# askerlee/AdaFace-dev

Measured on AMD Instinct MI355X. Metric: denoise-steps/sec SD-1.5 U-Net 512px bs=4/GPU, higher is better.
Workload: dtype f16; 1 GPU; adaface_txt2img_ddim: SD-1.5 U-Net eps-prediction + CFG + DDIM update, 512x512 (latent 64x64), bs=4/GPU, U-Net batch 8 (cond+uncond), 77 tokens, DDIM-50 timesteps, random-init weights; parallelism=replicas x1, hipgraph=True, finite=True

## Files before the change

adaface-dev_amd/csrc/af_attn.hip:

```cpp
#include <float.h>
#include <stdlib.h>

#include "af_common.h"

namespace {

struct AttnArgs {
  const half_t* q;
  const half_t* k;
  const half_t* vt;
  half_t* o;
  const float* kbias;
  float* lse2;
  int ld_lse;
  int causal_m;
  int B, Nq, L, heads, d;
  int ldq, ldk, ldo, ldv, ldb;
  long vbs;
  float c;
};

constexpr int KB = 64;
constexpr int VST = 36;
constexpr float kLazy = 8.0f;

template <int DS, bool ONES, bool GENERAL>
__global__ __launch_bounds__(256) void af_attn_kernel(AttnArgs a) {
  constexpr int DP = 16 * DS;
  constexpr int DT = (DS + 1) / 2;
  constexpr int DV = 32 * DT;
  constexpr int KST = DP + 8;
  constexpr int KBUF = KB * KST;
  constexpr int VBUF = 2 * DV * VST;
  constexpr int STAGE = KBUF + VBUF;
  constexpr int KCH = KB * (DP / 8);
  constexpr int NKC = (KCH + 255) / 256;
  constexpr int VCH = DV * 8;
  constexpr int NVC = (VCH + 255) / 256;
  extern __shared__ __attribute__((aligned(16))) char af_smem[];
  half_t* lds = reinterpret_cast<half_t*>(af_smem);

  const int tid = threadIdx.x, lane = tid & 63, wave = tid >> 6;
  const int r = lane & 31, hh = lane >> 5;
  const int qblocks = (a.Nq + 127) / 128;
  const int xcd = blockIdx.x & 7, idx = blockIdx.x >> 3;
  const int bh = (idx / qblocks) * 8 + xcd;
  if (bh >= a.B * a.heads) return;
  const int b = bh / a.heads, h = bh - b * a.heads;
  const int query = (idx % qblocks) * 128 + wave * 32 + r;


  half8_t qf[DS];
  const half8_t zero8 = {0, 0, 0, 0, 0, 0, 0, 0};
  {
    const half_t* qp = a.q + ((size_t)b * a.Nq + (query < a.Nq ? query : 0)) * a.ldq + h * a.d;
#pragma unroll
    for (int s = 0; s < DS; ++s) {
      const int dc = 16 * s + 8 * hh;
      half8_t v = (query < a.Nq && dc < a.d) ? *reinterpret_cast<const half8_t*>(qp + dc) : zero8;
#pragma unroll
      for (int e = 0; e < 8; ++e) v[e] = (half_t)((float)v[e] * a.c);
      qf[s] = v;
    }
  }

  half8_t rk[NKC], rv[NVC];
  const half_t* kptr[NKC];
  bool kok[NKC];
#pragma unroll
  for (int j = 0; j < NKC; ++j) {
    const int i = tid + 256 * j;
    const int row = i / (DP / 8), ch = i - row * (DP / 8);
    kok[j] = i < KCH && ch * 8 < a.d;
    kptr[j] = a.k + ((size_t)b * a.L + row) * a.ldk + h * a.d + ch * 8;
  }
  const half_t* vptr[NVC];
  bool vok[NVC], vones[NVC];
#pragma unroll
  for (int j = 0; j < NVC; ++j) {
    const int i = tid + 256 * j;
    const int row = i >> 3, ch = i & 7;
    vok[j] = i < VCH && row < a.d;
    vones[j] = ONES && i < VCH && row == DV - 1;
    vptr[j] = a.vt + (size_t)b * a.vbs + (size_t)(h * a.d + (row < a.d ? row : 0)) * a.ldv + ch * 8;
  }
  const half8_t ones8 = {1, 1, 1, 1, 1, 1, 1, 1};
  auto load_stage = [&](int key0) {
#pragma unroll
    for (int j = 0; j < NKC; ++j) {
      const int row = (tid + 256 * j) / (DP / 8);
      const bool ok = kok[j] && (!GENERAL || key0 + row < a.L);
      rk[j] = ok ? *reinterpret_cast<const half8_t*>(kptr[j] + (size_t)key0 * a.ldk) : zero8;
    }
#pragma unroll
    for (int j = 0; j < NVC; ++j) {
      const int kk = key0 + ((tid + 256 * j) & 7) * 8;
      const bool ok = vok[j] && (!GENERAL || kk < a.L);
      half8_t fill = zero8;
      if (ONES) {
        if (GENERAL) {
          if (vones[j]) {
#pragma unroll
            for (int e = 0; e < 8; ++e) fill[e] = (kk + e < a.L) ? (half_t)1 : (half_t)0;
          }
        } else {
          fill = vones[j] ? ones8 : zero8;
        }
      }
      rv[j] = ok ? *reinterpret_cast<const half8_t*>(vptr[j] + key0) : fill;
    }
  };
  auto store_stage = [&](int buf, int key0_store) {
    half_t* Ks = lds + buf * STAGE;
    half_t* Vs = Ks + KBUF;
#pragma unroll
    for (int j = 0; j < NKC; ++j) {
      const int i = tid + 256 * j;
      if (i < KCH) {
        const int row = i / (DP / 8), ch = i - row * (DP / 8);
        *reinterpret_cast<half8_t*>(Ks + row * KST + ch * 8) = rk[j];
      }
    }
#pragma unroll
    for (int j = 0; j < NVC; ++j) {
      const int i = tid + 256 * j;
      if (i < VCH) {
        const int row = i >> 3, ch = i & 7;
        half_t* dst = Vs + ((ch >> 2) * DV + row) * VST + (ch & 3) * 8;
        if (GENERAL) {
          const int kk = key0_store + ch * 8;
          if (kk + 8 > a.L) {
#pragma unroll
            for (int e = 0; e < 8; ++e)
              if (kk + e >= a.L) rv[j][e] = (half_t)0;
          }
        }
        const half4_t lo = {rv[j][0], rv[j][1], rv[j][2], rv[j][3]};
        const half4_t hi = {rv[j][4], rv[j][5], rv[j][6], rv[j][7]};
        *reinterpret_cast<half4_t*>(dst) = lo;
        *reinterpret_cast<half4_t*>(dst + 4) = hi;
      }
    }
  };

  floatx16 o[DT];
#pragma unroll
  for (int t = 0; t < DT; ++t)
#pragma unroll
    for (int i = 0; i < 16; ++i) o[t][i] = 0.f;
  float m = -FLT_MAX, l = 0.f;

  const int nstage = (a.L + KB - 1) / KB;
  load_stage(0);
  store_stage(0, 0);
  __syncthreads();
  for (int st = 0; st < nstage; ++st) {
    const int key0 = st * KB;
    const bool more = st + 1 < nstage;
    if (more) load_stage(key0 + KB);

    const half_t* Ks = lds + (st & 1) * STAGE;
    const half_t* Vs = Ks + KBUF;
    const int nsub = GENERAL ? ((key0 + 32 < a.L) ? 2 : 1) : 2;

    floatx16 sT[2];
    const float cinit = (GENERAL || st == 0) ? 0.f : -m;
#pragma unroll
    for (int sub = 0; sub < 2; ++sub) {
#pragma unroll
      for (int i = 0; i < 16; ++i) sT[sub][i] = cinit;
      if (sub < nsub) {
#pragma unroll
        for (int s = 0; s < DS; ++s) {
          const half8_t kf = *reinterpret_cast<const half8_t*>(Ks + (sub * 32 + r) * KST + 16 * s + 8 * hh);
          sT[sub] = __builtin_amdgcn_mfma_f32_32x32x16_f16(kf, qf[s], sT[sub], 0, 0, 0);
        }
      }
    }
    float mx = -FLT_MAX;
    if (GENERAL) {
#pragma unroll
      for (int sub = 0; sub < 2; ++sub) {
        if (sub < nsub) {
#pragma unroll
          for (int g = 0; g < 4; ++g) {
            const int kb = key0 + sub * 32 + 8 * g + 4 * hh;
            floatx4 bias = {0.f, 0.f, 0.f, 0.f};
            if (a.kbias) bias = *reinterpret_cast<const floatx4*>(a.kbias + (size_t)b * a.ldb + kb);
#pragma unroll
            for (int e = 0; e < 4; ++e) {
              float t = sT[sub][4 * g + e] + bias[e];
              bool vis = kb + e < a.L;
              if (a.causal_m > 0) vis = vis && ((kb + e) / a.causal_m <= query);
              t = vis ? t : -INFINITY;
              sT[sub][4 * g + e] = t;
              mx = fmaxf(mx, t);
            }
          }
        }
      }
    } else {
#pragma unroll
      for (int i = 0; i < 16; i += 2) {
        mx = fmaxf(fmaxf(mx, sT[0][i]), sT[0][i + 1]);
        mx = fmaxf(fmaxf(mx, sT[1][i]), sT[1][i + 1]);
      }
    }
    mx = fmaxf(mx, __shfl_xor(mx, 32, 64));
    if (GENERAL) {
      if (__builtin_amdgcn_ballot_w64(mx > m) != 0) {
        const float m_new = fmaxf(m, mx);
        const float alpha = __builtin_amdgcn_exp2f(m - m_new);
        m = m_new;
        if (!ONES) l *= alpha;
#pragma unroll
        for (int t = 0; t < DT; ++t)
#pragma unroll
          for (int i = 0; i < 16; ++i) o[t][i] *= alpha;
      }
      sT[0] = sT[0] - m;
      sT[1] = sT[1] - m;
    } else if (st == 0) {
      m = mx;
      sT[0] = sT[0] - m;
      sT[1] = sT[1] - m;
    } else if (__builtin_amdgcn_ballot_w64(mx > kLazy) != 0) {
      const float delta = fmaxf(mx, 0.f);
      const float alpha = __builtin_amdgcn_exp2f(-delta);
      m += delta;
      if (!ONES) l *= alpha;
#pragma unroll
      for (int t = 0; t < DT; ++t)
#pragma unroll
        for (int i = 0; i < 16; ++i) o[t][i] *= alpha;
      sT[0] = sT[0] - delta;
      sT[1] = sT[1] - delta;
    }

    half8_t pf[2][2];
#pragma unroll
    for (int sub = 0; sub < 2; ++sub) {
      if (sub < nsub) {
#pragma unroll
        for (int s2 = 0; s2 < 2; ++s2) {
#pragma unroll
          for (int j = 0; j < 8; ++j) {
            const float p = __builtin_amdgcn_exp2f(sT[sub][8 * s2 + j]);
            if (!ONES) l += p;
            pf[sub][s2][j] = (half_t)p;
          }
        }
      } else {
        pf[sub][0] = zero8;
        pf[sub][1] = zero8;
      }
    }
#pragma unroll
    for (int t = 0; t < DT; ++t) {
#pragma unroll
      for (int sub = 0; sub < 2; ++sub) {
        if (sub < nsub) {
#pragma unroll
          for (int s2 = 0; s2 < 2; ++s2) {
            const half_t* vp = Vs + (sub * DV + 32 * t + r) * VST + 16 * s2 + 4 * hh;
            const half4_t lo = *reinterpret_cast<const half4_t*>(vp);
            const half4_t hi = *reinterpret_cast<const half4_t*>(vp + 8);
            const half8_t vf = {lo[0], lo[1], lo[2], lo[3], hi[0], hi[1], hi[2], hi[3]};
            o[t] = __builtin_amdgcn_mfma_f32_32x32x16_f16(vf, pf[sub][s2], o[t], 0, 0, 0);
          }
        }
      }
    }

    if (more) store_stage((st + 1) & 1, key0 + KB);
    __syncthreads();
  }

  if (ONES) {
    const float mine = o[DT - 1][15];
    const float other = __shfl_xor(mine, 32, 64);
    l = hh ? mine : other;
  } else {
    l += __shfl_xor(l, 32, 64);
  }
  const float inv = 1.0f / l;
  if (a.lse2 && query < a.Nq && hh == 0) a.lse2[((size_t)b * a.heads + h) * a.ld_lse + query] = m + __builtin_amdgcn_logf(l);
  if (query < a.Nq) {
    half_t* op = a.o + ((size_t)b * a.Nq + query) * a.ldo + h * a.d;
#pragma unroll
    for (int t = 0; t < DT; ++t) {
#pragma unroll
      for (int g = 0; g < 4; ++g) {
        const int dd = 32 * t + 8 * g + 4 * hh;
        if (dd < a.d) {
          const half4_t v = {(half_t)(o[t][4 * g + 0] * inv), (half_t)(o[t][4 * g + 1] * inv),
                             (half_t)(o[t][4 * g + 2] * inv), (half_t)(o[t][4 * g + 3] * inv)};
          *reinterpret_cast<half4_t*>(op + dd) = v;
        }
      }
    }
  }
}

template <int DS, bool ONES, bool SLOT = false, int NW = 4>
__global__ __launch_bounds__(64 * NW) void af_attn2_kernel(AttnArgs a) {
  constexpr int NT = 64 * NW;
  constexpr int DP = 16 * DS, DT = (DS + 1) / 2, DV = 32 * DT;
  constexpr int KST = DP + 8, KBUF = KB * KST, VBUF = 2 * DV * VST, STAGE = KBUF + VBUF;
  constexpr int KCH = KB * (DP / 8), NKC = (KCH + NT - 1) / NT, VCH = DV * 8, NVC = (VCH + NT - 1) / NT;
  extern __shared__ __attribute__((aligned(16))) char af_smem[];
  half_t* lds = reinterpret_cast<half_t*>(af_smem);
  const int tid = threadIdx.x, lane = tid & 63, wave = tid >> 6;
  const int r = lane & 31, hh = lane >> 5;
  const int qblocks = (a.Nq + NT - 1) / NT;
  const int xcd = blockIdx.x & 7, idx = blockIdx.x >> 3;
  const int bh = (idx / qblocks) * 8 + xcd;
  if (bh >= a.B * a.heads) return;
  const int b = bh / a.heads, h = bh - b * a.heads;
  const int q0 = (idx % qblocks) * NT + wave * 64 + r;
  const half8_t zero8 = {0, 0, 0, 0, 0, 0, 0, 0};

  half8_t qf[2][DS];
#pragma unroll
  for (int c = 0; c < 2; ++c) {
    const int query = q0 + 32 * c;
    const half_t* qp = a.q + ((size_t)b * a.Nq + (query < a.Nq ? query : 0)) * a.ldq + h * a.d;
#pragma unroll
    for (int s = 0; s < DS; ++s) {
      const int dc = 16 * s + 8 * hh;
      half8_t v = (query < a.Nq && dc < a.d) ? *reinterpret_cast<const half8_t*>(qp + dc) : zero8;
#pragma unroll
      for (int e = 0; e < 8; ++e) v[e] = (half_t)((float)v[e] * a.c);
      qf[c][s] = v;
    }
  }

  half8_t rk[NKC], rv[NVC];
  const half_t* kptr[NKC];
  bool kok[NKC], kone[NKC];
#pragma unroll
  for (int j = 0; j < NKC; ++j) {
    const int i = tid + NT * j;
    const int row = i / (DP / 8), ch = i - row * (DP / 8);
    kok[j] = i < KCH && ch * 8 < a.d;
    kone[j] = SLOT && i < KCH && ch * 8 == a.d;
    kptr[j] = a.k + ((size_t)b * a.L + row) * a.ldk + h * a.d + ch * 8;
  }
  const half8_t one1 = {1, 0, 0, 0, 0, 0, 0, 0};
  const half_t* vptr[NVC];
  bool vok[NVC], vones[NVC];
#pragma unroll
  for (int j = 0; j < NVC; ++j) {
    const int i = tid + NT * j;
    const int row = i >> 3, ch = i & 7;
    vok[j] = i < VCH && row < a.d;
    vones[j] = ONES && i < VCH && row == DV - 1;
    vptr[j] = a.vt + (size_t)b * a.vbs + (size_t)(h * a.d + (row < a.d ? row : 0)) * a.ldv + ch * 8;
  }
  const half8_t ones8 = {1, 1, 1, 1, 1, 1, 1, 1};
  auto load_stage = [&](int key0) {
#pragma unroll
    for (int j = 0; j < NKC; ++j) rk[j] = kok[j] ? *reinterpret_cast<const half8_t*>(kptr[j] + (size_t)key0 * a.ldk) : (kone[j] ? one1 : zero8);
#pragma unroll
    for (int j = 0; j < NVC; ++j) rv[j] = vok[j] ? *reinterpret_cast<const half8_t*>(vptr[j] + key0) : (vones[j] ? ones8 : zero8);
  };
  auto store_stage = [&](int buf) {
    half_t* Ks = lds + buf * STAGE;
    half_t* Vs = Ks + KBUF;
#pragma unroll
    for (int j = 0; j < NKC; ++j) {
      const int i = tid + NT * j;
      if (i < KCH) {
        const int row = i / (DP / 8), ch = i - row * (DP / 8);
        *reinterpret_cast<half8_t*>(Ks + row * KST + ch * 8) = rk[j];
      }
    }
#pragma unroll
    for (int j = 0; j < NVC; ++j) {
      const int i = tid + NT * j;
      if (i < VCH) {
        const int row = i >> 3, ch = i & 7;
        half_t* dst = Vs + ((ch >> 2) * DV + row) * VST + (ch & 3) * 8;
        const half4_t lo = {rv[j][0], rv[j][1], rv[j][2], rv[j][3]};
        const half4_t hi = {rv[j][4], rv[j][5], rv[j][6], rv[j][7]};
        *reinterpret_cast<half4_t*>(dst) = lo;
        *reinterpret_cast<half4_t*>(dst + 4) = hi;
      }
    }
  };

  floatx16 o[2][DT];
#pragma unroll
  for (int c = 0; c < 2; ++c)
#pragma unroll
    for (int t = 0; t < DT; ++t)
#pragma unroll
      for (int i = 0; i < 16; ++i) o[c][t][i] = 0.f;
  float m[2] = {-FLT_MAX, -FLT_MAX}, l[2] = {0.f, 0.f};

  auto softmax = [&](int c, int st, floatx16 (&sT)[2], half8_t (&pf)[2][2]) {
    float mx = -FLT_MAX;
#pragma unroll
    for (int i = 0; i < 16; i += 2) {
      mx = fmaxf(fmaxf(mx, sT[0][i]), sT[0][i + 1]);
      mx = fmaxf(fmaxf(mx, sT[1][i]), sT[1][i + 1]);
    }
    if constexpr (SLOT) {
      const unsigned mb = __builtin_bit_cast(unsigned, mx);
      const auto sw = __builtin_amdgcn_permlane32_swap(mb, mb, false, false);
      mx = fmaxf(__builtin_bit_cast(float, (unsigned)sw[0]), __builtin_bit_cast(float, (unsigned)sw[1]));
    } else {
      mx = fmaxf(mx, __shfl_xor(mx, 32, 64));
    }
    if (st == 0) {
      const float m0 = SLOT ? (float)(half_t)mx : mx;
      m[c] = m0;
      sT[0] = sT[0] - m0;
      sT[1] = sT[1] - m0;
      if (SLOT && hh) qf[c][DS - 1][0] = (half_t)(-m0);
    } else if (__builtin_amdgcn_ballot_w64(mx > kLazy) != 0) {
      float delta = fmaxf(mx, 0.f);
      if constexpr (SLOT) {
        const float mn = (float)(half_t)(m[c] + delta);
        delta = mn - m[c];
        if (hh) qf[c][DS - 1][0] = (half_t)(-mn);
      }
      const float alpha = __builtin_amdgcn_exp2f(-delta);
      m[c] += delta;
      if (!ONES) l[c] *= alpha;
#pragma unroll
      for (int t = 0; t < DT; ++t)
#pragma unroll
        for (int i = 0; i < 16; ++i) o[c][t][i] *= alpha;
      sT[0] = sT[0] - delta;
      sT[1] = sT[1] - delta;
    }
#pragma unroll
    for (int sub = 0; sub < 2; ++sub)
#pragma unroll
      for (int s2 = 0; s2 < 2; ++s2)
#pragma unroll
        for (int j = 0; j < 8; ++j) {
          const float p = __builtin_amdgcn_exp2f(sT[sub][8 * s2 + j]);
          if (!ONES) l[c] += p;
          pf[sub][s2][j] = (half_t)p;
        }
  };

  const int nstage = a.L / KB;
  load_stage(0);
  store_stage(0);
  __syncthreads();
  if (NW == 8 && __builtin_amdgcn_readfirstlane(wave) >= 4) __builtin_amdgcn_s_setprio(1);
  for (int st = 0; st < nstage; ++st) {
    const bool more = st + 1 < nstage;
    if (more) load_stage((st + 1) * KB);
    const half_t* Ks = lds + (st & 1) * STAGE;
    const half_t* Vs = Ks + KBUF;

    floatx16 sA[2], sB[2];
    const floatx16 zero16 = {0.f, 0.f, 0.f, 0.f, 0.f, 0.f, 0.f, 0.f, 0.f, 0.f, 0.f, 0.f, 0.f, 0.f, 0.f, 0.f};
    if constexpr (!SLOT) {
      const float ca = st == 0 ? 0.f : -m[0], cb = st == 0 ? 0.f : -m[1];
#pragma unroll
      for (int sub = 0; sub < 2; ++sub) {
#pragma unroll
        for (int i = 0; i < 16; ++i) {
          sA[sub][i] = ca;
          sB[sub][i] = cb;
        }
      }
    }
#pragma unroll
    for (int sub = 0; sub < 2; ++sub)
#pragma unroll
      for (int s = 0; s < DS; ++s) {
        const half8_t kf = *reinterpret_cast<const half8_t*>(Ks + (sub * 32 + r) * KST + 16 * s + 8 * hh);
        sA[sub] = __builtin_amdgcn_mfma_f32_32x32x16_f16(kf, qf[0][s], (SLOT && s == 0) ? zero16 : sA[sub], 0, 0, 0);
      }
#pragma unroll
    for (int sub = 0; sub < 2; ++sub)
#pragma unroll
      for (int s = 0; s < DS; ++s) {
        const half8_t kf = *reinterpret_cast<const half8_t*>(Ks + (sub * 32 + r) * KST + 16 * s + 8 * hh);
        sB[sub] = __builtin_amdgcn_mfma_f32_32x32x16_f16(kf, qf[1][s], (SLOT && s == 0) ? zero16 : sB[sub], 0, 0, 0);
      }
    half8_t pA[2][2], pB[2][2];
    softmax(0, st, sA, pA);
#pragma unroll
    for (int t = 0; t < DT; ++t)
#pragma unroll
      for (int sub = 0; sub < 2; ++sub)
#pragma unroll
        for (int s2 = 0; s2 < 2; ++s2) {
          const half_t* vp = Vs + (sub * DV + 32 * t + r) * VST + 16 * s2 + 4 * hh;
          const half4_t lo = *reinterpret_cast<const half4_t*>(vp);
          const half4_t hi = *reinterpret_cast<const half4_t*>(vp + 8);
          const half8_t vf = {lo[0], lo[1], lo[2], lo[3], hi[0], hi[1], hi[2], hi[3]};
          o[0][t] = __builtin_amdgcn_mfma_f32_32x32x16_f16(vf, pA[sub][s2], o[0][t], 0, 0, 0);
        }
    softmax(1, st, sB, pB);
#pragma unroll
    for (int t = 0; t < DT; ++t)
#pragma unroll
      for (int sub = 0; sub < 2; ++sub)
#pragma unroll
        for (int s2 = 0; s2 < 2; ++s2) {
          const half_t* vp = Vs + (sub * DV + 32 * t + r) * VST + 16 * s2 + 4 * hh;
          const half4_t lo = *reinterpret_cast<const half4_t*>(vp);
          const half4_t hi = *reinterpret_cast<const half4_t*>(vp + 8);
          const half8_t vf = {lo[0], lo[1], lo[2], lo[3], hi[0], hi[1], hi[2], hi[3]};
          o[1][t] = __builtin_amdgcn_mfma_f32_32x32x16_f16(vf, pB[sub][s2], o[1][t], 0, 0, 0);
        }
    if (more) store_stage((st + 1) & 1);
    __syncthreads();
  }

#pragma unroll
  for (int c = 0; c < 2; ++c) {
    const int query = q0 + 32 * c;
    float lc = l[c];
    if (ONES) {
      const float mine = o[c][DT - 1][15];
      const float other = __shfl_xor(mine, 32, 64);
      lc = hh ? mine : other;
    } else {
      lc += __shfl_xor(lc, 32, 64);
    }
    const float inv = 1.0f / lc;
    if (a.lse2 && query < a.Nq && hh == 0) a.lse2[((size_t)b * a.heads + h) * a.ld_lse + query] = m[c] + __builtin_amdgcn_logf(lc);
    if (query < a.Nq) {
      half_t* op = a.o + ((size_t)b * a.Nq + query) * a.ldo + h * a.d;
#pragma unroll
      for (int t = 0; t < DT; ++t)
#pragma unroll
        for (int g = 0; g < 4; ++g) {
          const int dd = 32 * t + 8 * g + 4 * hh;
          if (dd < a.d) {
            const half4_t v = {(half_t)(o[c][t][4 * g + 0] * inv), (half_t)(o[c][t][4 * g + 1] * inv),
                               (half_t)(o[c][t][4 * g + 2] * inv), (half_t)(o[c][t][4 * g + 3] * inv)};
            *reinterpret_cast<half4_t*>(op + dd) = v;
          }
        }
    }
  }
}

template <int DS, bool ONES, bool SLOT = false>
int launch_attn2chain(const AttnArgs& a, hipStream_t stream) {
  constexpr int DP = 16 * DS, DT = (DS + 1) / 2, DV = 32 * DT;
  constexpr size_t lds = (size_t)2 * (KB * (DP + 8) + 2 * DV * VST) * sizeof(half_t);
  const int bh8 = (a.B * a.heads + 7) / 8 * 8;
  constexpr int kDefaultNw = 8;
  const char* nw_s = getenv("AF_ATTN_NW");
  const int nw = nw_s ? atoi(nw_s) : kDefaultNw;
  if (nw == 8 && SLOT && a.Nq % 512 == 0) {
    static bool attr8 = false;
    if (!af_allow_dyn_lds(reinterpret_cast<const void*>(&af_attn2_kernel<DS, ONES, SLOT, 8>), lds, attr8, "af_attention")) return af_check_launch("af_attention");
    hipLaunchKernelGGL((af_attn2_kernel<DS, ONES, SLOT, 8>), dim3((a.Nq / 512) * bh8), dim3(512), lds, stream, a);
    return af_check_launch("af_attention(two-chain, 8 waves)");
  }
  static bool attr_set = false;
  if (!af_allow_dyn_lds(reinterpret_cast<const void*>(&af_attn2_kernel<DS, ONES, SLOT>), lds, attr_set, "af_attention")) return af_check_launch("af_attention");
  const int qblocks = (a.Nq + 255) / 256;
  hipLaunchKernelGGL((af_attn2_kernel<DS, ONES, SLOT>), dim3(qblocks * bh8), dim3(256), lds, stream, a);
  return af_check_launch("af_attention(two-chain)");
}

template <int DS, bool ONES>
__global__ __launch_bounds__(256) void af_xattn_kernel(AttnArgs a, int groups_per_wave, int nchunk) {
  constexpr int DP = 16 * DS, DT = (DS + 1) / 2, DV = 32 * DT;
  constexpr int KST = DP + 8;
  constexpr int LP = 128;
  constexpr int KCH = LP * (DP / 8);
  constexpr int VCH = DV * (LP / 8);
  extern __shared__ __attribute__((aligned(16))) char af_smem[];
  half_t* Ks = reinterpret_cast<half_t*>(af_smem);
  half_t* Vs = Ks + LP * KST;

  const int tid = threadIdx.x, lane = tid & 63, wave = tid >> 6;
  const int r = lane & 31, hh = lane >> 5;
  const int xcd = blockIdx.x & 7, idx = blockIdx.x >> 3;
  const int bh = (idx / nchunk) * 8 + xcd;
  if (bh >= a.B * a.heads) return;
  const int chunk = idx % nchunk;
  const int b = bh / a.heads, h = bh - b * a.heads;

  const int nsub = (a.L + 31) >> 5;
  const half8_t zero8 = {0, 0, 0, 0, 0, 0, 0, 0};

  const int group0 = (chunk * 4 + wave) * groups_per_wave;
  auto load_q = [&](int grp, half8_t (&qf)[DS]) {
    const int query = grp * 32 + r;
    const half_t* qp = a.q + ((size_t)b * a.Nq + (query < a.Nq ? query : 0)) * a.ldq + h * a.d;
#pragma unroll
    for (int s2 = 0; s2 < DS; ++s2) {
      const int dc = 16 * s2 + 8 * hh;
      qf[s2] = (query < a.Nq && dc < a.d) ? *reinterpret_cast<const half8_t*>(qp + dc) : zero8;
    }
  };
  half8_t qraw[DS], qnext[DS];
  load_q(group0, qraw);

  {
    constexpr int NKC = (KCH + 255) / 256, NVC = (VCH + 255) / 256;
    half8_t rk[NKC], rv[NVC];
#pragma unroll
    for (int j = 0; j < NKC; ++j) {
      const int i = tid + 256 * j;
      const int row = i / (DP / 8), ch = i - row * (DP / 8);
      rk[j] = (i < KCH && row < a.L && ch * 8 < a.d)
                  ? *reinterpret_cast<const half8_t*>(a.k + ((size_t)b * a.L + row) * a.ldk + h * a.d + ch * 8) : zero8;
    }
#pragma unroll
    for (int j = 0; j < NVC; ++j) {
      const int i = tid + 256 * j;
      const int row = i >> 4, kk = (i & 15) * 8;
      rv[j] = (i < VCH && row < a.d && kk < a.L)
                  ? *reinterpret_cast<const half8_t*>(a.vt + (size_t)b * a.vbs + (size_t)(h * a.d + row) * a.ldv + kk) : zero8;
    }
#pragma unroll
    for (int j = 0; j < NKC; ++j) {
      const int i = tid + 256 * j;
      const int row = i / (DP / 8), ch = i - row * (DP / 8);
      if (i < KCH) *reinterpret_cast<half8_t*>(Ks + row * KST + ch * 8) = rk[j];
    }
#pragma unroll
    for (int j = 0; j < NVC; ++j) {
      const int i = tid + 256 * j;
      if (i < VCH) {
        const int row = i >> 4, ch = i & 15, kk = ch * 8;
        half8_t v = rv[j];
        if (row < a.d) {
          if (kk < a.L && kk + 8 > a.L) {
#pragma unroll
            for (int e = 0; e < 8; ++e)
              if (kk + e >= a.L) v[e] = (half_t)0;
          }
        } else if (ONES && row == DV - 1) {
#pragma unroll
          for (int e = 0; e < 8; ++e) v[e] = (kk + e < a.L) ? (half_t)1 : (half_t)0;
        }
        half_t* dst = Vs + ((ch >> 2) * DV + row) * VST + (ch & 3) * 8;
        const half4_t lo = {v[0], v[1], v[2], v[3]}, hi = {v[4], v[5], v[6], v[7]};
        *reinterpret_cast<half4_t*>(dst) = lo;
        *reinterpret_cast<half4_t*>(dst + 4) = hi;
      }
    }
  }
  __syncthreads();

  for (int gi = 0; gi < groups_per_wave; ++gi) {
    const int grp = group0 + gi;
    if (grp * 32 >= a.Nq) break;
    const int query = grp * 32 + r;
    if (gi + 1 < groups_per_wave) load_q(grp + 1, qnext);
    half8_t qf[DS];
#pragma unroll
    for (int s2 = 0; s2 < DS; ++s2)
#pragma unroll
      for (int e = 0; e < 8; ++e) qf[s2][e] = (half_t)((float)qraw[s2][e] * a.c);

    auto score_tile = [&](int sub) {
      floatx16 sc;
#pragma unroll
      for (int i = 0; i < 16; ++i) sc[i] = 0.f;
#pragma unroll
      for (int s2 = 0; s2 < DS; ++s2) {
        const half8_t kf = *reinterpret_cast<const half8_t*>(Ks + (sub * 32 + r) * KST + 16 * s2 + 8 * hh);
        sc = __builtin_amdgcn_mfma_f32_32x32x16_f16(kf, qf[s2], sc, 0, 0, 0);
      }
      if (sub == nsub - 1) {
#pragma unroll
        for (int i = 0; i < 16; ++i) {
          const int key = sub * 32 + 8 * (i >> 2) + 4 * hh + (i & 3);
          if (key >= a.L) sc[i] = -INFINITY;
        }
      }
      return sc;
    };
    float mx = -FLT_MAX;
#pragma unroll 1
    for (int sub = 0; sub < nsub; ++sub) {
      const floatx16 sc = score_tile(sub);
#pragma unroll
      for (int i = 0; i < 16; i += 2) mx = fmaxf(fmaxf(mx, sc[i]), sc[i + 1]);
    }
    mx = fmaxf(mx, __shfl_xor(mx, 32, 64));
    floatx16 o[DT];
#pragma unroll
    for (int t = 0; t < DT; ++t)
#pragma unroll
      for (int i = 0; i < 16; ++i) o[t][i] = 0.f;
    float l = 0.f;
#pragma unroll 1
    for (int sub = 0; sub < nsub; ++sub) {
      const floatx16 sc = score_tile(sub);
      half8_t pf[2];
#pragma unroll
      for (int s2 = 0; s2 < 2; ++s2)
#pragma unroll
        for (int j = 0; j < 8; ++j) {
          const float pv = __builtin_amdgcn_exp2f(sc[8 * s2 + j] - mx);
          if (!ONES) l += pv;
          pf[s2][j] = (half_t)pv;
        }
#pragma unroll
      for (int t = 0; t < DT; ++t)
#pragma unroll
        for (int s2 = 0; s2 < 2; ++s2) {
          const half_t* vp = Vs + (sub * DV + 32 * t + r) * VST + 16 * s2 + 4 * hh;
          const half4_t lo = *reinterpret_cast<const half4_t*>(vp);
          const half4_t hi = *reinterpret_cast<const half4_t*>(vp + 8);
          const half8_t vf = {lo[0], lo[1], lo[2], lo[3], hi[0], hi[1], hi[2], hi[3]};
          o[t] = __builtin_amdgcn_mfma_f32_32x32x16_f16(vf, pf[s2], o[t], 0, 0, 0);
        }
    }
    if (ONES) {
      const float mine = o[DT - 1][15];
      const float other = __shfl_xor(mine, 32, 64);
      l = hh ? mine : other;
    } else {
      l += __shfl_xor(l, 32, 64);
    }
    const float inv = 1.0f / l;
    if (a.lse2 && query < a.Nq && hh == 0) a.lse2[((size_t)b * a.heads + h) * a.ld_lse + query] = mx + __builtin_amdgcn_logf(l);
    if (query < a.Nq) {
      half_t* op = a.o + ((size_t)b * a.Nq + query) * a.ldo + h * a.d;
#pragma unroll
      for (int t = 0; t < DT; ++t)
#pragma unroll
        for (int g = 0; g < 4; ++g) {
          const int dd = 32 * t + 8 * g + 4 * hh;
          if (dd < a.d) {
            const half4_t v = {(half_t)(o[t][4 * g + 0] * inv), (half_t)(o[t][4 * g + 1] * inv),
                               (half_t)(o[t][4 * g + 2] * inv), (half_t)(o[t][4 * g + 3] * inv)};
            *reinterpret_cast<half4_t*>(op + dd) = v;
          }
        }
    }
    if (gi + 1 < groups_per_wave) {
#pragma unroll
      for (int s2 = 0; s2 < DS; ++s2) qraw[s2] = qnext[s2];
    }
  }
}

template <int DS, bool ONES>
int launch_xattn(const AttnArgs& a, hipStream_t stream) {
  constexpr int DP = 16 * DS, DT = (DS + 1) / 2, DV = 32 * DT;
  constexpr size_t lds = (size_t)(128 * (DP + 8) + 4 * DV * VST) * sizeof(half_t);
  static bool attr_set = false;
  if (!af_allow_dyn_lds(reinterpret_cast<const void*>(&af_xattn_kernel<DS, ONES>), lds, attr_set, "af_attention")) return af_check_launch("af_attention");
  const int groups = (a.Nq + 31) / 32;
  int gpw = groups / 32;
  gpw = gpw < 1 ? 1 : (gpw > 8 ? 8 : gpw);
  const int nchunk = (groups + 4 * gpw - 1) / (4 * gpw);
  const int bh8 = (a.B * a.heads + 7) / 8 * 8;
  hipLaunchKernelGGL((af_xattn_kernel<DS, ONES>), dim3(nchunk * bh8), dim3(256), lds, stream, a, gpw, nchunk);
  return af_check_launch("af_attention(short-key)");
}

template <int DS, bool ONES, bool GENERAL>
int launch_attn2(const AttnArgs& a, hipStream_t stream) {
  constexpr int DP = 16 * DS, DT = (DS + 1) / 2, DV = 32 * DT;
  constexpr size_t lds = (size_t)2 * (KB * (DP + 8) + 2 * DV * VST) * sizeof(half_t);
  static bool attr_set = false;
  if (!af_allow_dyn_lds(reinterpret_cast<const void*>(&af_attn_kernel<DS, ONES, GENERAL>), lds, attr_set, "af_attention")) return af_check_launch("af_attention");
  const int qblocks = (a.Nq + 127) / 128, bh8 = (a.B * a.heads + 7) / 8 * 8;
  dim3 grid(qblocks * bh8), block(256);
  hipLaunchKernelGGL((af_attn_kernel<DS, ONES, GENERAL>), grid, block, lds, stream, a);
  return af_check_launch("af_attention");
}

template <int DS>
int launch_attn(const AttnArgs& a, hipStream_t stream) {
  constexpr int DV = 32 * ((DS + 1) / 2);
  if (a.kbias == nullptr && a.causal_m == 0 && a.L <= 128)
    return DV > a.d ? launch_xattn<DS, true>(a, stream) : launch_xattn<DS, false>(a, stream);
  const bool general = a.kbias != nullptr || a.causal_m > 0 || a.L % KB != 0;
  if constexpr (DS <= 3) {
    if (!general && a.Nq >= 512) {
      if (a.d == 16 * DS - 8 && DV > a.d) return launch_attn2chain<DS, true, true>(a, stream);
      return DV > a.d ? launch_attn2chain<DS, true>(a, stream) : launch_attn2chain<DS, false>(a, stream);
    }
  }
  if (DV > a.d) return general ? launch_attn2<DS, true, true>(a, stream) : launch_attn2<DS, true, false>(a, stream);
  return general ? launch_attn2<DS, false, true>(a, stream) : launch_attn2<DS, false, false>(a, stream);
}

__global__ __launch_bounds__(256) void af_scores_kernel(const half_t* __restrict__ q, const half_t* __restrict__ k,
                                                        float* __restrict__ score, float* __restrict__ prob, int B, int Nq,
                                                        int L, int heads, int d, float scale) {
  const int lane = threadIdx.x & 63;
  const long row = (long)blockIdx.x * 4 + (threadIdx.x >> 6);
  const long nrows = (long)B * heads * Nq;
  if (row >= nrows) return;
  const int i = (int)(row % Nq);
  const int h = (int)((row / Nq) % heads);
  const int b = (int)(row / ((long)Nq * heads));
  const int C = heads * d;
  const half_t* qp = q + ((size_t)b * Nq + i) * C + h * d;
  float s[2];
#pragma unroll
  for (int jj = 0; jj < 2; ++jj) {
    const int j = lane + 64 * jj;
    float acc = 0.f;
    if (j < L) {
      const half_t* kp = k + ((size_t)b * L + j) * C + h * d;
      for (int c0 = 0; c0 < d; c0 += 8) {
        const half8_t qv = *reinterpret_cast<const half8_t*>(qp + c0);
        const half8_t kv = *reinterpret_cast<const half8_t*>(kp + c0);
#pragma unroll
        for (int e = 0; e < 8; ++e) acc += (float)qv[e] * (float)kv[e];
      }
    }
    s[jj] = j < L ? acc * scale : -INFINITY;
  }
  const float mx = af_wave_max(fmaxf(s[0], s[1]));
  const float e0 = __expf(s[0] - mx), e1 = __expf(s[1] - mx);
  const float inv = 1.0f / af_wave_sum(e0 + e1);
  float* sp = score + (size_t)row * L;
  float* pp = prob + (size_t)row * L;
  if (lane < L) {
    sp[lane] = s[0];
    pp[lane] = e0 * inv;
  }
  if (lane + 64 < L) {
    sp[lane + 64] = s[1];
    pp[lane + 64] = e1 * inv;
  }
}

}

extern "C" int af_attention_lse(const void* q, const void* k, const void* vt, void* o, void* lse2, int ld_lse,
                                const void* keybias, int B, int Nq, int L, int heads, int d, int ldq, int ldk, int ldo,
                                int ldv, int ldb, float scale, void* stream) {
  return af_attention_ex(q, k, vt, o, lse2, ld_lse, keybias, 0, B, Nq, L, heads, d, ldq, ldk, ldo, ldv, ldb, scale, stream);
}

extern "C" int af_attention_strided(const void* q, const void* k, const void* vt, void* o, void* lse2, int ld_lse, const void* keybias,
                                    int causal_m, int B, int Nq, int L, int heads, int d, int ldq, int ldk, int ldo, int ldv, int ldb,
                                    int64_t vt_batch_stride, float scale, void* stream);

extern "C" int af_attention_ex(const void* q, const void* k, const void* vt, void* o, void* lse2, int ld_lse,
                               const void* keybias, int causal_m, int B, int Nq, int L, int heads, int d, int ldq, int ldk,
                               int ldo, int ldv, int ldb, float scale, void* stream) {
  return af_attention_strided(q, k, vt, o, lse2, ld_lse, keybias, causal_m, B, Nq, L, heads, d, ldq, ldk, ldo, ldv, ldb,
                              (int64_t)heads * d * ldv, scale, stream);
}

extern "C" int af_attention_strided(const void* q, const void* k, const void* vt, void* o, void* lse2, int ld_lse, const void* keybias,
                                    int causal_m, int B, int Nq, int L, int heads, int d, int ldq, int ldk, int ldo, int ldv, int ldb,
                                    int64_t vt_batch_stride, float scale, void* stream) {
  AF_REQUIRE(q && k && vt && o, "af_attention: null pointer");
  AF_REQUIRE(vt_batch_stride >= (int64_t)heads * d * ldv && vt_batch_stride % 8 == 0, "af_attention: vt_batch_stride must cover heads*d rows of ldv and keep 16-byte alignment");
  AF_REQUIRE(B > 0 && Nq > 0 && L > 0 && heads > 0 && d > 0, "af_attention: bad sizes");
  AF_REQUIRE(d % 8 == 0, "af_attention: head dim must be a multiple of 8");
  AF_SUPPORTED(d <= 160, "af_attention: head dim > 160");
  const int C = heads * d;
  AF_REQUIRE(ldq >= C && ldk >= C && ldo >= C && ldq % 8 == 0 && ldk % 8 == 0 && ldo % 4 == 0,
             "af_attention: bad row strides");
  AF_REQUIRE(ldv % 8 == 0 && ldv >= ((L + 7) / 8) * 8, "af_attention: ldv must be a multiple of 8 and >= roundup(L, 8)");
  if (keybias) AF_REQUIRE(ldb >= ((L + KB - 1) / KB) * KB && ldb % 4 == 0, "af_attention: ldb must cover L rounded up to 64");
  AttnArgs a;
  a.q = (const half_t*)q;
  a.k = (const half_t*)k;
  a.vt = (const half_t*)vt;
  a.o = (half_t*)o;
  a.kbias = (const float*)keybias;
  a.lse2 = (float*)lse2;
  a.ld_lse = ld_lse;
  a.causal_m = causal_m;
  AF_REQUIRE(causal_m >= 0, "af_attention: causal_m < 0");
  if (lse2) AF_REQUIRE(ld_lse >= Nq, "af_attention: ld_lse < Nq");
  a.B = B;
  a.Nq = Nq;
  a.L = L;
  a.heads = heads;
  a.d = d;
  a.ldq = ldq;
  a.ldk = ldk;
  a.ldo = ldo;
  a.ldv = ldv;
  a.ldb = ldb;
  a.vbs = vt_batch_stride;
  a.c = scale * 1.4426950408889634f;
  AfLaunchScope scope(L < Nq ? AF_FAM_XATTN : AF_FAM_ATTN, stream);
  hipStream_t s = (hipStream_t)stream;
  const int ds = (d + 15) / 16;
  switch (ds) {
    case 1: return launch_attn<1>(a, s);
    case 2: return launch_attn<2>(a, s);
    case 3: return launch_attn<3>(a, s);
    case 4: return launch_attn<4>(a, s);
    case 5: return launch_attn<5>(a, s);
    case 6: return launch_attn<6>(a, s);
    case 8: return launch_attn<8>(a, s);
    case 10: return launch_attn<10>(a, s);
    default: return af_fail(AF_E_UNSUPPORTED, "af_attention: unsupported head dim (need ceil(d/16) in {1,2,3,4,5,6,8,10})");
  }
}

extern "C" int af_attention(const void* q, const void* k, const void* vt, void* o, const void* keybias, int B, int Nq,
                            int L, int heads, int d, int ldq, int ldk, int ldo, int ldv, int ldb, float scale,
                            void* stream) {
  return af_attention_lse(q, k, vt, o, nullptr, 0, keybias, B, Nq, L, heads, d, ldq, ldk, ldo, ldv, ldb, scale, stream);
}

extern "C" int af_attention_scores(const void* q, const void* k, void* score, void* prob, int B, int Nq, int L, int heads,
                                   int d, float scale, void* stream) {
  AF_REQUIRE(q && k && score && prob, "af_attention_scores: null pointer");
  AF_REQUIRE(B > 0 && Nq > 0 && L > 0 && heads > 0 && d > 0 && d % 8 == 0, "af_attention_scores: bad sizes");
  AF_SUPPORTED(L <= 128, "af_attention_scores: L > 128 (capture path is for cross-attention only)");
  const long rows = (long)B * heads * Nq;
  dim3 grid((unsigned)((rows + 3) / 4)), block(256);
  AfLaunchScope scope(AF_FAM_ATTN, stream);
  hipLaunchKernelGGL(af_scores_kernel, grid, block, 0, (hipStream_t)stream, (const half_t*)q, (const half_t*)k,
                     (float*)score, (float*)prob, B, Nq, L, heads, d, scale);
  return af_check_launch("af_attention_scores");
}
```

adaface-dev_amd/csrc/af_common.h:

```cpp
#pragma once
#include <hip/hip_runtime.h>
#include <stdint.h>
#include <stdlib.h>
#include <string>

#include "../../include/adaface_hip.h"

typedef _Float16 half_t;
typedef _Float16 half2_t __attribute__((ext_vector_type(2)));
typedef _Float16 half4_t __attribute__((ext_vector_type(4)));
typedef _Float16 half8_t __attribute__((ext_vector_type(8)));
typedef float floatx4 __attribute__((ext_vector_type(4)));
typedef unsigned int uintx4_t __attribute__((ext_vector_type(4)));
typedef float floatx16 __attribute__((ext_vector_type(16)));

#define AF_WAVE 64

void af_set_error(const std::string& msg);
int af_fail(int code, const std::string& msg);

struct AfLaunchScope {
  int family;
  hipStream_t stream;
  hipEvent_t ev_stop;
  unsigned epoch;
  AfLaunchScope(int family, void* stream);
  ~AfLaunchScope();
};
int af_check_launch(const char* what);
bool af_allow_dyn_lds(const void* kernel, size_t bytes, bool& done, const char* what);
void af_launch_transpose_tokens(const _Float16* x, _Float16* y, int B, int N, int C, int ldx, int ldy, hipStream_t stream);
struct AfTransposeJob {
  const _Float16* x;
  _Float16* y;
  int N, C, ldx, ldy;
};
void af_launch_transpose_tokens_multi(const AfTransposeJob* jobs, int n, int B, hipStream_t stream);

#define AF_REQUIRE(cond, msg)                                      \
  do {                                                             \
    if (!(cond)) return af_fail(AF_E_BADARG, std::string(msg));    \
  } while (0)
#define AF_SUPPORTED(cond, msg)                                      \
  do {                                                               \
    if (!(cond)) return af_fail(AF_E_UNSUPPORTED, std::string(msg)); \
  } while (0)

__device__ __forceinline__ float af_sigmoid(float x) { return __builtin_amdgcn_rcpf(1.0f + __expf(-x)); }
__device__ __forceinline__ float af_silu(float x) { return x * af_sigmoid(x); }
__device__ __forceinline__ float af_erf(float x) {
  const float ax = fabsf(x);
  const float t = __builtin_amdgcn_rcpf(fmaf(0.3275911f, ax, 1.0f));
  float p = fmaf(1.061405429f, t, -1.453152027f);
  p = fmaf(p, t, 1.421413741f);
  p = fmaf(p, t, -0.284496736f);
  p = fmaf(p, t, 0.254829592f);
  const float e = __builtin_amdgcn_exp2f(ax * ax * -1.4426950408889634f);
  return copysignf(fmaf(-p * t, e, 1.0f), x);
}
__device__ __forceinline__ float af_gelu_erf(float x) { return 0.5f * x * (1.0f + af_erf(x * 0.70710678118654752f)); }

__device__ __forceinline__ float af_wave_sum(float v) {
#pragma unroll
  for (int off = 32; off > 0; off >>= 1) v += __shfl_xor(v, off, 64);
  return v;
}
__device__ __forceinline__ float af_wave_max(float v) {
#pragma unroll
  for (int off = 32; off > 0; off >>= 1) v = fmaxf(v, __shfl_xor(v, off, 64));
  return v;
}

struct GnAcc {
  float n, s, m2;
};
__device__ __forceinline__ GnAcc gn_acc_merge(const GnAcc a, const GnAcc b) {
  if (b.n <= 0.f) return a;
  if (a.n <= 0.f) return b;
  const float n = a.n + b.n;
  const float d = b.s * __builtin_amdgcn_rcpf(b.n) - a.s * __builtin_amdgcn_rcpf(a.n);
  GnAcc r;
  r.n = n;
  r.s = a.s + b.s;
  r.m2 = a.m2 + b.m2 + d * d * (a.n * b.n * __builtin_amdgcn_rcpf(n));
  return r;
}
__device__ __forceinline__ GnAcc gn_acc_from_shifted(float n, float p, float s1, float q1) {
  GnAcc r;
  r.n = n;
  r.s = n * p + s1;
  r.m2 = n > 0.f ? fmaxf(q1 - s1 * s1 * __builtin_amdgcn_rcpf(n), 0.f) : 0.f;
  return r;
}

__device__ __forceinline__ half2_t gn_half_diff(const half2_t x, const half2_t nhp) {
  const half2_t h = {(half_t)0.5f, (half_t)0.5f};
  return x * h + nhp;
}

constexpr int AF_WPF_MAX = 8;
constexpr int AF_WPF_DUMP_BYTES = 256;
struct AfWpf {
  int budget, coop;
};
inline AfWpf af_wpf_config(int tiles_m) {
  static const int budget_env = getenv("AF_GEMM3_WPREFETCH") ? atoi(getenv("AF_GEMM3_WPREFETCH")) : 4;
  static const int coop_env = getenv("AF_GEMM3_WPF_COOP") ? atoi(getenv("AF_GEMM3_WPF_COOP")) : 32;
  return AfWpf{budget_env > AF_WPF_MAX ? AF_WPF_MAX : budget_env, tiles_m < coop_env ? tiles_m : coop_env};
}
__device__ __forceinline__ void af_prefetch_weight_tile(const half_t* wt, int kpad, int npad, int row0, int rows, int kt0, int nk, int coop, int me,
                                                        int budget, int nw, int wave, int lane, char* lds_dump) {
  const int total = rows * nk;
  const int per = (total + coop - 1) / coop;
  const int begin = me * per;
  const int end = min(total, begin + min(per, budget * nw * 64));
#pragma unroll
  for (int j = 0; j < AF_WPF_MAX; ++j) {
    const int line = begin + (j * nw + wave) * 64 + lane;
    if (j < budget && line < end) {
      const int st = line / rows, row = line - st * rows;
      const int n = row0 + row;
      if (n < npad)
        __builtin_amdgcn_global_load_lds((const __attribute__((address_space(1))) void*)(wt + (size_t)n * kpad + (size_t)(kt0 + st) * 64),
                                         (__attribute__((address_space(3))) void*)lds_dump, 4, 0, 0);
    }
  }
}
```

adaface-dev_amd/csrc/af_runtime.hip:

```cpp
#include <atomic>
#include <mutex>
#include <vector>

#include "af_common.h"

static thread_local std::string g_last_error;

void af_set_error(const std::string& msg) { g_last_error = msg; }
int af_fail(int code, const std::string& msg) {
  g_last_error = msg;
  return code;
}

extern "C" const char* af_last_error(void) { return g_last_error.c_str(); }
extern "C" int af_version(void) { return 100; }

extern "C" int af_device_count(void) {
  int n = 0;
  hipError_t e = hipGetDeviceCount(&n);
  if (e != hipSuccess) return af_fail(AF_E_HIP, std::string("hipGetDeviceCount: ") + hipGetErrorString(e));
  return n;
}

static thread_local std::string g_pending_error;

bool af_allow_dyn_lds(const void* kernel, size_t bytes, bool& done, const char* what) {
  if (done || bytes <= 65536) return true;
  hipError_t e = hipFuncSetAttribute(kernel, hipFuncAttributeMaxDynamicSharedMemorySize, (int)bytes);
  if (e != hipSuccess) {
    (void)hipGetLastError();
    g_pending_error = std::string(what) + ": hipFuncSetAttribute(MaxDynamicSharedMemorySize = " + std::to_string(bytes) + "): " + hipGetErrorString(e);
    return false;
  }
  done = true;
  return true;
}

int af_check_launch(const char* what) {
  if (!g_pending_error.empty()) {
    std::string m;
    m.swap(g_pending_error);
    (void)hipGetLastError();
    return af_fail(AF_E_HIP, m);
  }
  hipError_t e = hipGetLastError();
  if (e != hipSuccess) return af_fail(AF_E_HIP, std::string(what) + ": " + hipGetErrorString(e));
  return AF_OK;
}

namespace {
struct ProfState {
  std::mutex mu;
  std::atomic<bool> on{false};
  unsigned epoch = 0;
  struct Pair {
    hipEvent_t a, b;
  };
  std::vector<Pair> pairs[AF_FAM_COUNT];
  std::vector<Pair> pool;
};
ProfState& prof() {
  static ProfState s;
  return s;
}
}

AfLaunchScope::AfLaunchScope(int family_, void* stream_) : family(family_), stream((hipStream_t)stream_), ev_stop(nullptr), epoch(0) {
  ProfState& p = prof();
  if (!p.on.load(std::memory_order_relaxed)) return;
  hipStreamCaptureStatus cs = hipStreamCaptureStatusNone;
  if (hipStreamIsCapturing(stream, &cs) != hipSuccess || cs != hipStreamCaptureStatusNone) return;
  std::lock_guard<std::mutex> lk(p.mu);
  ProfState::Pair pr;
  if (!p.pool.empty()) {
    pr = p.pool.back();
    p.pool.pop_back();
  } else {
    if (hipEventCreate(&pr.a) != hipSuccess) return;
    if (hipEventCreate(&pr.b) != hipSuccess) {
      (void)hipEventDestroy(pr.a);
      return;
    }
  }
  (void)hipEventRecord(pr.a, stream);
  p.pairs[family].push_back(pr);
  ev_stop = pr.b;
  epoch = p.epoch;
}

AfLaunchScope::~AfLaunchScope() {
  if (!ev_stop) return;
  ProfState& p = prof();
  std::lock_guard<std::mutex> lk(p.mu);
  if (epoch != p.epoch) return;
  (void)hipEventRecord(ev_stop, stream);
}

extern "C" int af_prof_enable(int on) {
  ProfState& p = prof();
  p.on.store(on != 0);
  return AF_OK;
}

extern "C" int af_prof_reset(void) {
  ProfState& p = prof();
  std::lock_guard<std::mutex> lk(p.mu);
  ++p.epoch;
  for (int f = 0; f < AF_FAM_COUNT; ++f) {
    for (auto& pr : p.pairs[f]) p.pool.push_back(pr);
    p.pairs[f].clear();
  }
  return AF_OK;
}

extern "C" int af_prof_read(int family, int* launches, double* total_ms) {
  if (family < 0 || family >= AF_FAM_COUNT || !launches || !total_ms) return af_fail(AF_E_BADARG, "af_prof_read: bad argument");
  ProfState& p = prof();
  std::lock_guard<std::mutex> lk(p.mu);
  double tot = 0.0;
  for (auto& pr : p.pairs[family]) {
    hipError_t e = hipEventSynchronize(pr.b);
    if (e != hipSuccess) return af_fail(AF_E_HIP, std::string("hipEventSynchronize: ") + hipGetErrorString(e));
    float ms = 0.f;
    e = hipEventElapsedTime(&ms, pr.a, pr.b);
    if (e != hipSuccess) return af_fail(AF_E_HIP, std::string("hipEventElapsedTime: ") + hipGetErrorString(e));
    tot += ms;
  }
  *launches = (int)p.pairs[family].size();
  *total_ms = tot;
  return AF_OK;
}
```

Baseline: 100.1 denoise-steps/s.

## Add key-group multi-stage LDS buffering and reuse V fragments across query chains

Adds an optional attention kernel variant that stages several key blocks per barrier and prefetches K fragments into registers. It is selectable through AF_ATTN_KGROUP and defaults to off. In the default path, V fragments read from LDS for the first query chain are now kept in registers and reused for the second chain, halving V LDS reads. The trade-off is higher register pressure, which may reduce occupancy or cause spills.

```diff
diff --git a/adaface-dev_amd/csrc/af_attn.hip b/adaface-dev_amd/csrc/af_attn.hip
--- a/adaface-dev_amd/csrc/af_attn.hip
+++ b/adaface-dev_amd/csrc/af_attn.hip
@@ -1,5 +1,7 @@
 #include <float.h>
 #include <stdlib.h>
+
+#include <type_traits>
 
 #include "af_common.h"
 
@@ -302,8 +304,9 @@
   }
 }
 
-template <int DS, bool ONES, bool SLOT = false, int NW = 4>
+template <int DS, bool ONES, bool SLOT = false, int NW = 4, int KG = 1>
 __global__ __launch_bounds__(64 * NW) void af_attn2_kernel(AttnArgs a) {
+  static_assert(KG == 1 || KG == 2 || KG == 4, "key groups of 1, 2 or 4 sub-stages");
   constexpr int NT = 64 * NW;
   constexpr int DP = 16 * DS, DT = (DS + 1) / 2, DV = 32 * DT;
   constexpr int KST = DP + 8, KBUF = KB * KST, VBUF = 2 * DV * VST, STAGE = KBUF + VBUF;
@@ -398,7 +401,7 @@
       for (int i = 0; i < 16; ++i) o[c][t][i] = 0.f;
   float m[2] = {-FLT_MAX, -FLT_MAX}, l[2] = {0.f, 0.f};
 
-  auto softmax = [&](int c, int st, floatx16 (&sT)[2], half8_t (&pf)[2][2]) {
+  auto softmax = [&](int c, auto first, floatx16 (&sT)[2], half8_t (&pf)[2][2]) {
     float mx = -FLT_MAX;
 #pragma unroll
     for (int i = 0; i < 16; i += 2) {
@@ -412,7 +415,7 @@
     } else {
       mx = fmaxf(mx, __shfl_xor(mx, 32, 64));
     }
-    if (st == 0) {
+    if (first) {
       const float m0 = SLOT ? (float)(half_t)mx : mx;
       m[c] = m0;
       sT[0] = sT[0] - m0;
@@ -448,20 +451,24 @@
   };
 
   const int nstage = a.L / KB;
-  load_stage(0);
-  store_stage(0);
-  __syncthreads();
-  if (NW == 8 && __builtin_amdgcn_readfirstlane(wave) >= 4) __builtin_amdgcn_s_setprio(1);
-  for (int st = 0; st < nstage; ++st) {
-    const bool more = st + 1 < nstage;
-    if (more) load_stage((st + 1) * KB);
-    const half_t* Ks = lds + (st & 1) * STAGE;
+  auto read_kf = [&](int buf, half8_t (&kf)[2][DS]) {
+    const half_t* Ks = lds + buf * STAGE;
+#pragma unroll
+    for (int sub = 0; sub < 2; ++sub)
+#pragma unroll
+      for (int s = 0; s < DS; ++s) kf[sub][s] = *reinterpret_cast<const half8_t*>(Ks + (sub * 32 + r) * KST + 16 * s + 8 * hh);
+  };
+  auto substage = [&](auto first, int buf, int nxt, int wbuf, half8_t (&kf)[2][DS], bool ahead) __attribute__((always_inline)) {
+    constexpr bool have_kf = KG > 1;
+    const bool more = nxt < nstage;
+    if (more) load_stage(nxt * KB);
+    const half_t* Ks = lds + buf * STAGE;
     const half_t* Vs = Ks + KBUF;
 
     floatx16 sA[2], sB[2];
     const floatx16 zero16 = {0.f, 0.f, 0.f, 0.f, 0.f, 0.f, 0.f, 0.f, 0.f, 0.f, 0.f, 0.f, 0.f, 0.f, 0.f, 0.f};
     if constexpr (!SLOT) {
-      const float ca = st == 0 ? 0.f : -m[0], cb = st == 0 ? 0.f : -m[1];
+      const float ca = first ? 0.f : -m[0], cb = first ? 0.f : -m[1];
 #pragma unroll
       for (int sub = 0; sub < 2; ++sub) {
 #pragma unroll
@@ -475,18 +482,19 @@
     for (int sub = 0; sub < 2; ++sub)
 #pragma unroll
       for (int s = 0; s < DS; ++s) {
-        const half8_t kf = *reinterpret_cast<const half8_t*>(Ks + (sub * 32 + r) * KST + 16 * s + 8 * hh);
-        sA[sub] = __builtin_amdgcn_mfma_f32_32x32x16_f16(kf, qf[0][s], (SLOT && s == 0) ? zero16 : sA[sub], 0, 0, 0);
+        const half8_t kfa = have_kf ? kf[sub][s] : *reinterpret_cast<const half8_t*>(Ks + (sub * 32 + r) * KST + 16 * s + 8 * hh);
+        sA[sub] = __builtin_amdgcn_mfma_f32_32x32x16_f16(kfa, qf[0][s], (SLOT && s == 0) ? zero16 : sA[sub], 0, 0, 0);
       }
 #pragma unroll
     for (int sub = 0; sub < 2; ++sub)
 #pragma unroll
       for (int s = 0; s < DS; ++s) {
-        const half8_t kf = *reinterpret_cast<const half8_t*>(Ks + (sub * 32 + r) * KST + 16 * s + 8 * hh);
-        sB[sub] = __builtin_amdgcn_mfma_f32_32x32x16_f16(kf, qf[1][s], (SLOT && s == 0) ? zero16 : sB[sub], 0, 0, 0);
+        const half8_t kfb = have_kf ? kf[sub][s] : *reinterpret_cast<const half8_t*>(Ks + (sub * 32 + r) * KST + 16 * s + 8 * hh);
+        sB[sub] = __builtin_amdgcn_mfma_f32_32x32x16_f16(kfb, qf[1][s], (SLOT && s == 0) ? zero16 : sB[sub], 0, 0, 0);
       }
     half8_t pA[2][2], pB[2][2];
-    softmax(0, st, sA, pA);
+    softmax(0, first, sA, pA);
+    half8_t vf[DT][2][2];
 #pragma unroll
     for (int t = 0; t < DT; ++t)
 #pragma unroll
@@ -496,24 +504,43 @@
           const half_t* vp = Vs + (sub * DV + 32 * t + r) * VST + 16 * s2 + 4 * hh;
           const half4_t lo = *reinterpret_cast<const half4_t*>(vp);
           const half4_t hi = *reinterpret_cast<const half4_t*>(vp + 8);
-          const half8_t vf = {lo[0], lo[1], lo[2], lo[3], hi[0], hi[1], hi[2], hi[3]};
-          o[0][t] = __builtin_amdgcn_mfma_f32_32x32x16_f16(vf, pA[sub][s2], o[0][t], 0, 0, 0);
-        }
-    softmax(1, st, sB, pB);
+          vf[t][sub][s2] = half8_t{lo[0], lo[1], lo[2], lo[3], hi[0], hi[1], hi[2], hi[3]};
+          o[0][t] = __builtin_amdgcn_mfma_f32_32x32x16_f16(vf[t][sub][s2], pA[sub][s2], o[0][t], 0, 0, 0);
+        }
+    if constexpr (have_kf) read_kf(ahead ? buf + 1 : buf, kf);
+    softmax(1, first, sB, pB);
 #pragma unroll
     for (int t = 0; t < DT; ++t)
 #pragma unroll
       for (int sub = 0; sub < 2; ++sub)
 #pragma unroll
-        for (int s2 = 0; s2 < 2; ++s2) {
-          const half_t* vp = Vs + (sub * DV + 32 * t + r) * VST + 16 * s2 + 4 * hh;
-          const half4_t lo = *reinterpret_cast<const half4_t*>(vp);
-          const half4_t hi = *reinterpret_cast<const half4_t*>(vp + 8);
-          const half8_t vf = {lo[0], lo[1], lo[2], lo[3], hi[0], hi[1], hi[2], hi[3]};
-          o[1][t] = __builtin_amdgcn_mfma_f32_32x32x16_f16(vf, pB[sub][s2], o[1][t], 0, 0, 0);
-        }
-    if (more) store_stage((st + 1) & 1);
-    __syncthreads();
+        for (int s2 = 0; s2 < 2; ++s2) o[1][t] = __builtin_amdgcn_mfma_f32_32x32x16_f16(vf[t][sub][s2], pB[sub][s2], o[1][t], 0, 0, 0);
+    if (more) store_stage(wbuf);
+  };
+
+  for (int j = 0; j < KG && (j == 0 || j < nstage); ++j) {
+    load_stage(j * KB);
+    store_stage(j);
+  }
+  __syncthreads();
+  if (NW == 8 && __builtin_amdgcn_readfirstlane(wave) >= 4) __builtin_amdgcn_s_setprio(1);
+  half8_t kf[2][DS];
+  if constexpr (KG == 1) {
+    for (int st = 0; st < nstage; ++st) {
+      substage(st == 0, st & 1, st + 1, (st + 1) & 1, kf, false);
+      __syncthreads();
+    }
+  } else {
+    read_kf(0, kf);
+    substage(std::true_type{}, 0, KG, KG, kf, nstage > 1);
+    for (int g0 = 0; g0 < nstage; g0 += KG) {
+      const int slot = (g0 / KG & 1) * KG;
+      const int nsub = nstage - g0 < KG ? nstage - g0 : KG;
+      if (g0 > 0) read_kf(slot, kf);
+#pragma unroll 1
+      for (int j = g0 > 0 ? 0 : 1; j < nsub; ++j) substage(std::false_type{}, slot + j, g0 + j + KG, (KG - slot) + j, kf, j + 1 < nsub);
+      __syncthreads();
+    }
   }
 
 #pragma unroll
@@ -546,15 +573,47 @@
   }
 }
 
+int attn_kgroup_override() {
+  static const int v = [] {
+    const char* s = getenv("AF_ATTN_KGROUP");
+    return s ? atoi(s) : 0;
+  }();
+  return v;
+}
+
+template <int DS, bool ONES, bool SLOT, int KG>
+bool try_attn2chain_groups(const AttnArgs& a, hipStream_t stream) {
+  constexpr int DP = 16 * DS, DT = (DS + 1) / 2, DV = 32 * DT;
+  constexpr size_t lds = (size_t)2 * KG * (KB * (DP + 8) + 2 * DV * VST) * sizeof(half_t);
+  static int granted = 0;
+  if (!af_try_dyn_lds(reinterpret_cast<const void*>(&af_attn2_kernel<DS, ONES, SLOT, 8, KG>), lds, granted)) return false;
+  hipLaunchKernelGGL((af_attn2_kernel<DS, ONES, SLOT, 8, KG>), dim3((a.Nq / 512) * ((a.B * a.heads + 7) / 8 * 8)), dim3(512), lds, stream, a);
+  return true;
+}
+
 template <int DS, bool ONES, bool SLOT = false>
 int launch_attn2chain(const AttnArgs& a, hipStream_t stream) {
   constexpr int DP = 16 * DS, DT = (DS + 1) / 2, DV = 32 * DT;
   constexpr size_t lds = (size_t)2 * (KB * (DP + 8) + 2 * DV * VST) * sizeof(half_t);
   const int bh8 = (a.B * a.heads + 7) / 8 * 8;
+  const int kg_env = attn_kgroup_override();
+  if (kg_env != 0 && kg_env != 1 && kg_env != 2 && kg_env != 4) return af_fail(AF_E_BADARG, "af_attention: AF_ATTN_KGROUP must be 1, 2 or 4");
   constexpr int kDefaultNw = 8;
+  constexpr int kDefaultKgroup = 1;
   const char* nw_s = getenv("AF_ATTN_NW");
   const int nw = nw_s ? atoi(nw_s) : kDefaultNw;
-  if (nw == 8 && SLOT && a.Nq % 512 == 0) {
+  const bool nw8 = nw == 8 && SLOT && a.Nq % 512 == 0;
+  if constexpr (SLOT && DS == 3) {
+    if (nw8) {
+      const int nstage = a.L / KB;
+      const int kg_max = kg_env ? kg_env : kDefaultKgroup;
+      bool done = false;
+      if (kg_max >= 4 && (kg_env || nstage >= 8)) done = try_attn2chain_groups<DS, ONES, SLOT, 4>(a, stream);
+      if (!done && kg_max >= 2 && (kg_env || nstage >= 4)) done = try_attn2chain_groups<DS, ONES, SLOT, 2>(a, stream);
+      if (done) return af_check_launch("af_attention(two-chain, 8 waves, key groups)");
+    }
+  }
+  if (nw8) {
     static bool attr8 = false;
     if (!af_allow_dyn_lds(reinterpret_cast<const void*>(&af_attn2_kernel<DS, ONES, SLOT, 8>), lds, attr8, "af_attention")) return af_check_launch("af_attention");
     hipLaunchKernelGGL((af_attn2_kernel<DS, ONES, SLOT, 8>), dim3((a.Nq / 512) * bh8), dim3(512), lds, stream, a);
diff --git a/adaface-dev_amd/csrc/af_common.h b/adaface-dev_amd/csrc/af_common.h
--- a/adaface-dev_amd/csrc/af_common.h
+++ b/adaface-dev_amd/csrc/af_common.h
@@ -29,6 +29,7 @@
 };
 int af_check_launch(const char* what);
 bool af_allow_dyn_lds(const void* kernel, size_t bytes, bool& done, const char* what);
+bool af_try_dyn_lds(const void* kernel, size_t bytes, int& state);
 void af_launch_transpose_tokens(const _Float16* x, _Float16* y, int B, int N, int C, int ldx, int ldy, hipStream_t stream);
 struct AfTransposeJob {
   const _Float16* x;
diff --git a/adaface-dev_amd/csrc/af_runtime.hip b/adaface-dev_amd/csrc/af_runtime.hip
--- a/adaface-dev_amd/csrc/af_runtime.hip
+++ b/adaface-dev_amd/csrc/af_runtime.hip
@@ -34,6 +34,14 @@
   }
   done = true;
   return true;
+}
+
+bool af_try_dyn_lds(const void* kernel, size_t bytes, int& state) {
+  if (state == 0) {
+    state = bytes <= 65536 || hipFuncSetAttribute(kernel, hipFuncAttributeMaxDynamicSharedMemorySize, (int)bytes) == hipSuccess ? 1 : -1;
+    if (state < 0) (void)hipGetLastError();
+  }
+  return state > 0;
 }
 
 int af_check_launch(const char* what) {
```

Result: no change. 100.8 denoise-steps/s (median of 6 runs) (+0.7%).
